# dlilien/ImpDAR

Measured on NVIDIA B200. Metric: migrated samples/s, higher is better.
Workload: dtype f32

## Files before the change

### impdar_b200/csrc/kirchhoff_tile.cuh

```cuda
#pragma once

namespace impdar {

#ifndef KT_CFG_NW
#define KT_CFG_NW 28
#endif
#ifndef KT_CFG_NP
#define KT_CFG_NP 4
#endif
#ifndef KT_CFG_RW
#define KT_CFG_RW 1
#endif
#ifndef KT_CFG_TR
#define KT_CFG_TR 8
#endif
#ifndef KT_CFG_W
#define KT_CFG_W 16
#endif
#ifndef KT_CFG_NST
#define KT_CFG_NST 4
#endif
constexpr int KT_NW = KT_CFG_NW;
constexpr int KT_NP = KT_CFG_NP;
constexpr int KT_RW = KT_CFG_RW;
constexpr int KT_Q = KT_NW * KT_RW;
constexpr int KT_TR = KT_CFG_TR;
constexpr int KT_X = 32 * KT_TR;
constexpr int KT_W = KT_CFG_W;
constexpr int KT_NST = KT_CFG_NST;
#ifndef KT_CFG_FLUSH
#define KT_CFG_FLUSH 4
#endif
constexpr int KT_FLUSH = KT_CFG_FLUSH;
constexpr int KT_SPAN = 120;
constexpr int KT_SEGW = KT_X + KT_SPAN + 8;
constexpr int KT_STAGE_FLOATS = KT_W * 2 * KT_SEGW;
constexpr int KT_RING = 33;
constexpr size_t KT_SMEM = (size_t)KT_NST * KT_STAGE_FLOATS * sizeof(float) +
                           (size_t)KT_NW * KT_RW * KT_RING * sizeof(int4) + 2 * KT_NST * sizeof(unsigned long long) + 16;
constexpr int KT_THREADS = (KT_NW + KT_NP) * 32;
constexpr int KT_RPP = (KT_W + KT_NP - 1) / KT_NP;
static_assert(KT_RPP <= 32 && KT_NW + KT_NP <= 32, "tile kernel configuration");

struct KirchTileParams {
    const int2 *seg;
    const int *nstage;
    int *sched_flags;
    int t_base;
};

struct KtPlace {
    long long gl, gr;
    unsigned nl, nr;
    int dl, dr;
    int ol, orr;
};
__device__ __forceinline__ KtPlace kt_place(const KirchTabParams &p, int x0, int k, int slot, int j, int2 e) {
    const int span = e.y - e.x;
    const long long rowoff = (long long)k * p.Tp + p.Apad + x0;
    const long long il = rowoff - e.y, ir = rowoff + e.x;
    const int shl = (int)(il & 3), shr = (int)(ir & 3);
    KtPlace r;
    r.gl = il - shl;
    r.gr = ir - shr;
    r.nl = (unsigned)((shl + KT_X + span + 3) & ~3);
    r.nr = (unsigned)((shr + KT_X + span + 3) & ~3);
    r.dl = slot * KT_STAGE_FLOATS + j * 2 * KT_SEGW;
    r.dr = r.dl + KT_SEGW;
    r.ol = r.dl + shl + e.y;
    r.orr = r.dr + shr - e.x;
    return r;
}

__device__ __forceinline__ unsigned kt_smem_u32(const void *p) { return (unsigned)__cvta_generic_to_shared(p); }
__device__ __forceinline__ void kt_mbar_init(unsigned long long *bar, int count) {
    asm volatile("mbarrier.init.shared::cta.b64 [%0], %1;" ::"r"(kt_smem_u32(bar)), "r"(count) : "memory");
}
__device__ __forceinline__ void kt_mbar_arrive(unsigned long long *bar) {
    asm volatile("mbarrier.arrive.shared::cta.b64 _, [%0];" ::"r"(kt_smem_u32(bar)) : "memory");
}
__device__ __forceinline__ void kt_mbar_arrive_tx(unsigned long long *bar, unsigned bytes) {
    asm volatile("mbarrier.arrive.expect_tx.shared::cta.b64 _, [%0], %1;" ::"r"(kt_smem_u32(bar)), "r"(bytes) : "memory");
}
#ifndef KT_CFG_SLEEP
#define KT_CFG_SLEEP 0
#endif
__device__ __forceinline__ bool kt_mbar_try(unsigned long long *bar, unsigned parity) {
    unsigned ok;
    asm volatile(
        "{\n"
        ".reg .pred p;\n"
        "mbarrier.try_wait.parity.shared::cta.b64 p, [%1], %2;\n"
        "selp.u32 %0, 1, 0, p;\n"
        "}\n"
        : "=r"(ok)
        : "r"(kt_smem_u32(bar)), "r"(parity)
        : "memory");
    return ok != 0;
}
__device__ __forceinline__ void kt_mbar_wait(unsigned long long *bar, unsigned parity) {
    while (!kt_mbar_try(bar, parity)) {
        if (KT_CFG_SLEEP) __nanosleep(KT_CFG_SLEEP);
    }
}
__device__ __forceinline__ void kt_bulk_load(void *smem_dst, const void *gsrc, unsigned bytes, unsigned long long *bar) {
    asm volatile("cp.async.bulk.shared::cluster.global.mbarrier::complete_tx::bytes [%0], [%1], %2, [%3];" ::"r"(
                     kt_smem_u32(smem_dst)),
                 "l"(gsrc), "r"(bytes), "r"(kt_smem_u32(bar))
                 : "memory");
}

__global__ void __launch_bounds__(256) kirch_tile_sched_kernel(const int2 *__restrict__ tab, const int *__restrict__ nm,
                                                               int S, int A1, int s_begin, int s_end, int2 *__restrict__ seg,
                                                               int *__restrict__ nstage, int *__restrict__ sched_flags) {
    __shared__ int s_kmax, s_wide;
    const int b = blockIdx.x;
    const int t0 = s_begin + b * KT_Q, t1 = min(t0 + KT_Q, s_end);
    int2 *__restrict__ sb = seg + (size_t)b * S;
    if (threadIdx.x == 0) { s_kmax = -1; s_wide = 0; }
    for (int k = t0 + threadIdx.x; k < S; k += blockDim.x) sb[k] = make_int2(0x7fffffff, -1);
    __syncthreads();
    int kmax = -1;
    for (int ti = t0; ti < t1; ++ti) {
        const int n = nm[ti];
        const int2 *__restrict__ row = tab + (size_t)ti * A1;
        for (int m = threadIdx.x; m < n; m += blockDim.x) {
            const int k = row[m].x;
            if (k >= 0) {
                atomicMin(&sb[k].x, m);
                atomicMax(&sb[k].y, m);
                kmax = max(kmax, k);
            }
        }
    }
    if (kmax >= 0) atomicMax(&s_kmax, kmax);
    __syncthreads();
    int wide = 0;
    for (int k = t0 + threadIdx.x; k < S; k += blockDim.x) {
        const int2 e = sb[k];
        if (e.y >= e.x && e.y - e.x > KT_SPAN) wide = 1;
    }
    if (wide) atomicOr(&s_wide, 1);
    __syncthreads();
    if (threadIdx.x == 0) {
        const int kbase = (t0 / KT_W) * KT_W;
        nstage[b] = s_kmax < 0 ? 0 : (s_kmax - kbase) / KT_W + 1;
        if (s_wide) atomicOr(sched_flags, 1);
    }
}

__global__ void __launch_bounds__(256) kirch_table_count_kernel(const int2 *__restrict__ tab, const int *__restrict__ nm,
                                                                int A1, int T, int x_begin, int x_end, int s_begin,
                                                                unsigned long long *__restrict__ stats) {
    const int ti = s_begin + blockIdx.x;
    const int n = nm[ti];
    const int2 *__restrict__ row = tab + (size_t)ti * A1;
    unsigned long long c = 0;
    for (int m = threadIdx.x; m < n; m += blockDim.x) {
        if (row[m].x < 0) continue;
        c += (unsigned long long)max(0, x_end - max(x_begin, m));
        if (m) c += (unsigned long long)max(0, min(x_end, T - m) - x_begin);
    }
#pragma unroll
    for (int o = 16; o > 0; o >>= 1) c += __shfl_xor_sync(0xffffffffu, c, o);
    if ((threadIdx.x & 31) == 0 && c) atomicAdd(&stats[0], c);
}

__global__ void __launch_bounds__(KT_THREADS, 1) kirch_tile_kernel(const __grid_constant__ KirchTabParams p,
                                                                   const __grid_constant__ KirchTileParams q) {
    extern __shared__ __align__(128) unsigned char kt_smem_raw[];
    if (q.sched_flags[0] != 0) return;
    const int b = blockIdx.x;
    const int t0 = q.t_base + b * KT_Q;
    const int r_lo = max(t0, p.flags[0]);
    if (min(t0 + KT_Q, p.s_end) <= r_lo) return;
    float *buf = reinterpret_cast<float *>(kt_smem_raw);
    int4 *rings = reinterpret_cast<int4 *>(buf + (size_t)KT_NST * KT_STAGE_FLOATS);
    unsigned long long *full = reinterpret_cast<unsigned long long *>(rings + KT_NW * KT_RW * KT_RING);
    unsigned long long *empty = full + KT_NST;

    const int x0 = p.x_begin + blockIdx.y * KT_X;
    const int nst = q.nstage[b];
    const int kbase = (t0 / KT_W) * KT_W;
    const int warp = threadIdx.x >> 5, lane = threadIdx.x & 31;
    const int2 *__restrict__ sb = q.seg + (size_t)b * p.S;

    if (threadIdx.x == 0) {
        for (int i = 0; i < KT_NST; ++i) {
            kt_mbar_init(&full[i], KT_NP);
            kt_mbar_init(&empty[i], KT_NW);
        }
        asm volatile("fence.mbarrier_init.release.cluster;" ::: "memory");
    }
    __syncthreads();

    if (warp >= KT_NW) {
        const int pw = warp - KT_NW;
        for (int s = 0; s < nst; ++s) {
            const int slot = s % KT_NST;
            if (s >= KT_NST) kt_mbar_wait(&empty[slot], (unsigned)((s / KT_NST - 1) & 1));
            unsigned bytes = 0, nl = 0, nr = 0;
            const float *gl = nullptr, *gr = nullptr;
            float *dl = nullptr, *dr = nullptr;
            const int j = pw * KT_RPP + lane;
            if (lane < KT_RPP && j < KT_W) {
                const int k = kbase + s * KT_W + j;
                int2 e = make_int2(1, 0);
                if (k >= t0 && k < p.S) e = sb[k];
                if (e.y >= e.x) {
                    const KtPlace pl = kt_place(p, x0, k, slot, j, e);
                    nl = pl.nl;
                    nr = pl.nr;
                    gl = p.gP + pl.gl;
                    gr = p.gP + pl.gr;
                    dl = buf + pl.dl;
                    dr = buf + pl.dr;
                    bytes = (nl + nr) * 4u;
                }
            }
            const unsigned total = __reduce_add_sync(0xffffffffu, bytes);
            __syncwarp();
            if (lane == 0) kt_mbar_arrive_tx(&full[slot], total);
            __syncwarp();
            if (bytes) {
                kt_bulk_load(dl, gl, nl * 4u, &full[slot]);
                kt_bulk_load(dr, gr, nr * 4u, &full[slot]);
            }
        }
        return;
    }

    float2 acc[KT_RW][KT_TR / 2], tot[KT_RW][KT_TR / 2];
    int mnext[KT_RW], mend[KT_RW];
    int pos[KT_RW], cnt[KT_RW];
    int csk[KT_RW];
    bool live[KT_RW];
    const int2 *trow[KT_RW];
    int2 pre[KT_RW];
    int4 *ring[KT_RW];
    int4 cur[KT_RW];
    const int2 none = make_int2(-1, 0);
    auto decode = [&](int w) {
        const int m = mnext[w] + lane;
        const int2 e = pre[w];
        pre[w] = m + 32 < mend[w] ? __ldg(trow[w] + m + 32) : none;
        const unsigned v = __ballot_sync(0xffffffffu, e.x >= 0);
        __syncwarp();
        csk[w] = 0x7fffffff;
        if (e.x >= 0) {
            const unsigned rel = (unsigned)(e.x - kbase), sk = rel / KT_W;
            const KtPlace pl = kt_place(p, x0, e.x, (int)(sk % KT_NST), (int)(rel % KT_W), __ldg(sb + e.x));
            const float wgt = __int_as_float(e.y) * (m == 0 ? 0.5f : 1.0f);
            ring[w][__popc(v & ((1u << lane) - 1u))] =
                make_int4((pl.ol - m) * 4, (pl.orr + m) * 4, __float_as_int(wgt), 0);
            csk[w] = (int)sk;
        }
        __syncwarp();
        mnext[w] += 32;
        pos[w] = 0;
        cnt[w] = __popc(v);
        cur[w] = ring[w][0];
    };
#pragma unroll
    for (int w = 0; w < KT_RW; ++w) {
        const int ti = t0 + warp + w * KT_NW;
        live[w] = ti >= max(p.s_begin, r_lo) && ti < p.s_end && (x0 < p.x_end);
        mnext[w] = 0;
        mend[w] = live[w] ? p.nm[ti] : 0;
        trow[w] = p.tab + (size_t)(live[w] ? ti : t0) * p.A1;
        ring[w] = rings + (size_t)(warp * KT_RW + w) * KT_RING;
        pre[w] = lane < mend[w] ? __ldg(trow[w] + lane) : none;
        decode(w);
#pragma unroll
        for (int r = 0; r < KT_TR / 2; ++r) acc[w][r] = tot[w][r] = make_float2(0.f, 0.f);
    }
    const char *__restrict__ lbuf = reinterpret_cast<const char *>(buf + lane);
    const int sabs0 = kbase / KT_W;
    for (int s = 0; s < nst; ++s) {
        const int slot = s % KT_NST;
        kt_mbar_wait(&full[slot], (unsigned)((s / KT_NST) & 1));
#pragma unroll
        for (int w = 0; w < KT_RW; ++w) {
            while (true) {
                const int end = __popc(__ballot_sync(0xffffffffu, csk[w] <= s));
                int4 d = cur[w];
#pragma unroll 1
                for (int i = pos[w]; i < end; ++i) {
                    const int4 nx = ring[w][i + 1];
                    const float *__restrict__ pl = reinterpret_cast<const float *>(lbuf + d.x);
                    const float *__restrict__ pr = reinterpret_cast<const float *>(lbuf + d.y);
                    const float wgt = __int_as_float(d.z);
                    const float2 w2 = make_float2(wgt, wgt);
#pragma unroll
                    for (int r = 0; r < KT_TR / 2; ++r) {
                        const float2 l = make_float2(pl[64 * r], pl[64 * r + 32]);
                        const float2 g = make_float2(pr[64 * r], pr[64 * r + 32]);
                        acc[w][r] = __ffma2_rn(w2, __fadd2_rn(l, g), acc[w][r]);
                    }
                    d = nx;
                }
                cur[w] = d;
                pos[w] = end;
                if (end < cnt[w] || mnext[w] >= mend[w]) break;
                decode(w);
            }
        }
        if (((sabs0 + s) & (KT_FLUSH - 1)) == KT_FLUSH - 1) {
#pragma unroll
            for (int w = 0; w < KT_RW; ++w)
#pragma unroll
                for (int r = 0; r < KT_TR / 2; ++r) {
                    tot[w][r] = __fadd2_rn(tot[w][r], acc[w][r]);
                    acc[w][r] = make_float2(0.f, 0.f);
                }
        }
        __syncwarp();
        if (lane == 0) kt_mbar_arrive(&empty[slot]);
    }
#pragma unroll
    for (int w = 0; w < KT_RW; ++w) {
        const int ti = t0 + warp + w * KT_NW;
        if (!live[w]) continue;
#pragma unroll
        for (int r = 0; r < KT_TR / 2; ++r) {
            const float2 v = __fadd2_rn(tot[w][r], acc[w][r]);
            const int x = x0 + lane + 64 * r;
            if (x < p.x_end) p.out[(size_t)ti * p.ldo + (x - p.x_begin)] = v.x;
            if (x + 32 < p.x_end) p.out[(size_t)ti * p.ldo + (x + 32 - p.x_begin)] = v.y;
        }
    }
}

}
```

Measured before the change: 3.523 billion.

## Pair adjacent output rows per warp to share identical shared-memory tap reads

Each consumer warp now handles two adjacent output traces (14 warps × 2 rows instead of 28 × 1). While decoding, it marks each tap entry whose trace index matches the neighbouring row's entry at the same offset. Matching taps are then processed together, with one shared-memory load feeding two FMAs, and non-matching runs are unrolled by two. This is meant to cut shared-memory bandwidth and instruction count per accumulation, at the cost of fewer warps for latency hiding, more register pressure and more complex control flow.

```diff
diff --git a/impdar_b200/csrc/kirchhoff_tile.cuh b/impdar_b200/csrc/kirchhoff_tile.cuh
--- a/impdar_b200/csrc/kirchhoff_tile.cuh
+++ b/impdar_b200/csrc/kirchhoff_tile.cuh
@@ -2,15 +2,9 @@
 
 namespace impdar {
 
-#ifndef KT_CFG_NW
-#define KT_CFG_NW 28
-#endif
 #ifndef KT_CFG_NP
 #define KT_CFG_NP 4
 #endif
-#ifndef KT_CFG_RW
-#define KT_CFG_RW 1
-#endif
 #ifndef KT_CFG_TR
 #define KT_CFG_TR 8
 #endif
@@ -20,10 +14,9 @@
 #ifndef KT_CFG_NST
 #define KT_CFG_NST 4
 #endif
-constexpr int KT_NW = KT_CFG_NW;
+constexpr int KT_NW = 14;
 constexpr int KT_NP = KT_CFG_NP;
-constexpr int KT_RW = KT_CFG_RW;
-constexpr int KT_Q = KT_NW * KT_RW;
+constexpr int KT_Q = 2 * KT_NW;
 constexpr int KT_TR = KT_CFG_TR;
 constexpr int KT_X = 32 * KT_TR;
 constexpr int KT_W = KT_CFG_W;
@@ -35,9 +28,9 @@
 constexpr int KT_SPAN = 120;
 constexpr int KT_SEGW = KT_X + KT_SPAN + 8;
 constexpr int KT_STAGE_FLOATS = KT_W * 2 * KT_SEGW;
-constexpr int KT_RING = 33;
+constexpr int KT_RING = 34;
 constexpr size_t KT_SMEM = (size_t)KT_NST * KT_STAGE_FLOATS * sizeof(float) +
-                           (size_t)KT_NW * KT_RW * KT_RING * sizeof(int4) + 2 * KT_NST * sizeof(unsigned long long) + 16;
+                           (size_t)KT_NW * 2 * KT_RING * sizeof(int4) + 2 * KT_NST * sizeof(unsigned long long) + 16;
 constexpr int KT_THREADS = (KT_NW + KT_NP) * 32;
 constexpr int KT_RPP = (KT_W + KT_NP - 1) / KT_NP;
 static_assert(KT_RPP <= 32 && KT_NW + KT_NP <= 32, "tile kernel configuration");
@@ -176,7 +169,7 @@
     if (min(t0 + KT_Q, p.s_end) <= r_lo) return;
     float *buf = reinterpret_cast<float *>(kt_smem_raw);
     int4 *rings = reinterpret_cast<int4 *>(buf + (size_t)KT_NST * KT_STAGE_FLOATS);
-    unsigned long long *full = reinterpret_cast<unsigned long long *>(rings + KT_NW * KT_RW * KT_RING);
+    unsigned long long *full = reinterpret_cast<unsigned long long *>(rings + KT_NW * 2 * KT_RING);
     unsigned long long *empty = full + KT_NST;
 
     const int x0 = p.x_begin + blockIdx.y * KT_X;
@@ -230,20 +223,23 @@
         return;
     }
 
-    float2 acc[KT_RW][KT_TR / 2], tot[KT_RW][KT_TR / 2];
-    int mnext[KT_RW], mend[KT_RW];
-    int pos[KT_RW], cnt[KT_RW];
-    int csk[KT_RW];
-    bool live[KT_RW];
-    const int2 *trow[KT_RW];
-    int2 pre[KT_RW];
-    int4 *ring[KT_RW];
-    int4 cur[KT_RW];
+    float2 acc[2][KT_TR / 2], tot[2][KT_TR / 2];
+    int mnext[2], mend[2];
+    int pos[2], cnt[2];
+    int csk[2];
+    const int2 *trow[2];
+    int2 pre[2];
+    int prek[2];
+    int4 *ring[2];
+    int4 cur[2];
+    bool live[2];
     const int2 none = make_int2(-1, 0);
     auto decode = [&](int w) {
         const int m = mnext[w] + lane;
         const int2 e = pre[w];
+        const int ko = prek[w];
         pre[w] = m + 32 < mend[w] ? __ldg(trow[w] + m + 32) : none;
+        prek[w] = m + 32 < mend[1 - w] ? __ldg(&trow[1 - w][m + 32].x) : -1;
         const unsigned v = __ballot_sync(0xffffffffu, e.x >= 0);
         __syncwarp();
         csk[w] = 0x7fffffff;
@@ -252,7 +248,7 @@
             const KtPlace pl = kt_place(p, x0, e.x, (int)(sk % KT_NST), (int)(rel % KT_W), __ldg(sb + e.x));
             const float wgt = __int_as_float(e.y) * (m == 0 ? 0.5f : 1.0f);
             ring[w][__popc(v & ((1u << lane) - 1u))] =
-                make_int4((pl.ol - m) * 4, (pl.orr + m) * 4, __float_as_int(wgt), 0);
+                make_int4((pl.ol - m) * 4, (pl.orr + m) * 4, __float_as_int(wgt), e.x == ko);
             csk[w] = (int)sk;
         }
         __syncwarp();
@@ -262,52 +258,99 @@
         cur[w] = ring[w][0];
     };
 #pragma unroll
-    for (int w = 0; w < KT_RW; ++w) {
-        const int ti = t0 + warp + w * KT_NW;
+    for (int w = 0; w < 2; ++w) {
+        const int ti = t0 + 2 * warp + w;
         live[w] = ti >= max(p.s_begin, r_lo) && ti < p.s_end && (x0 < p.x_end);
         mnext[w] = 0;
         mend[w] = live[w] ? p.nm[ti] : 0;
         trow[w] = p.tab + (size_t)(live[w] ? ti : t0) * p.A1;
-        ring[w] = rings + (size_t)(warp * KT_RW + w) * KT_RING;
+        ring[w] = rings + (size_t)(warp * 2 + w) * KT_RING;
+#pragma unroll
+        for (int r = 0; r < KT_TR / 2; ++r) acc[w][r] = tot[w][r] = make_float2(0.f, 0.f);
+    }
+#pragma unroll
+    for (int w = 0; w < 2; ++w) {
         pre[w] = lane < mend[w] ? __ldg(trow[w] + lane) : none;
+        prek[w] = lane < mend[1 - w] ? __ldg(&trow[1 - w][lane].x) : -1;
         decode(w);
-#pragma unroll
-        for (int r = 0; r < KT_TR / 2; ++r) acc[w][r] = tot[w][r] = make_float2(0.f, 0.f);
     }
     const char *__restrict__ lbuf = reinterpret_cast<const char *>(buf + lane);
     const int sabs0 = kbase / KT_W;
     for (int s = 0; s < nst; ++s) {
         const int slot = s % KT_NST;
         kt_mbar_wait(&full[slot], (unsigned)((s / KT_NST) & 1));
-#pragma unroll
-        for (int w = 0; w < KT_RW; ++w) {
-            while (true) {
-                const int end = __popc(__ballot_sync(0xffffffffu, csk[w] <= s));
-                int4 d = cur[w];
+        while (true) {
+            const int end0 = __popc(__ballot_sync(0xffffffffu, csk[0] <= s));
+            const int end1 = __popc(__ballot_sync(0xffffffffu, csk[1] <= s));
+            auto run = [&](int w, int end) {
+                int4 d = cur[w], nx = ring[w][pos[w] + 1];
+                int i = pos[w];
 #pragma unroll 1
-                for (int i = pos[w]; i < end; ++i) {
-                    const int4 nx = ring[w][i + 1];
+                while (i < end && !d.w) {
                     const float *__restrict__ pl = reinterpret_cast<const float *>(lbuf + d.x);
                     const float *__restrict__ pr = reinterpret_cast<const float *>(lbuf + d.y);
-                    const float wgt = __int_as_float(d.z);
-                    const float2 w2 = make_float2(wgt, wgt);
-#pragma unroll
-                    for (int r = 0; r < KT_TR / 2; ++r) {
-                        const float2 l = make_float2(pl[64 * r], pl[64 * r + 32]);
-                        const float2 g = make_float2(pr[64 * r], pr[64 * r + 32]);
-                        acc[w][r] = __ffma2_rn(w2, __fadd2_rn(l, g), acc[w][r]);
+                    const float2 w2 = make_float2(__int_as_float(d.z), __int_as_float(d.z));
+                    float2 lg[KT_TR / 2];
+#pragma unroll
+                    for (int r = 0; r < KT_TR / 2; ++r)
+                        lg[r] = __fadd2_rn(make_float2(pl[64 * r], pl[64 * r + 32]), make_float2(pr[64 * r], pr[64 * r + 32]));
+                    if (i + 1 < end && !nx.w) {
+                        const int4 n2 = ring[w][i + 2], n3 = ring[w][i + 3];
+                        const float *__restrict__ ql = reinterpret_cast<const float *>(lbuf + nx.x);
+                        const float *__restrict__ qr = reinterpret_cast<const float *>(lbuf + nx.y);
+                        const float2 v2 = make_float2(__int_as_float(nx.z), __int_as_float(nx.z));
+                        float2 lh[KT_TR / 2];
+#pragma unroll
+                        for (int r = 0; r < KT_TR / 2; ++r)
+                            lh[r] = __fadd2_rn(make_float2(ql[64 * r], ql[64 * r + 32]), make_float2(qr[64 * r], qr[64 * r + 32]));
+#pragma unroll
+                        for (int r = 0; r < KT_TR / 2; ++r) acc[w][r] = __ffma2_rn(w2, lg[r], acc[w][r]);
+#pragma unroll
+                        for (int r = 0; r < KT_TR / 2; ++r) acc[w][r] = __ffma2_rn(v2, lh[r], acc[w][r]);
+                        d = n2;
+                        nx = n3;
+                        i += 2;
+                    } else {
+                        const int4 n2 = ring[w][i + 2];
+#pragma unroll
+                        for (int r = 0; r < KT_TR / 2; ++r) acc[w][r] = __ffma2_rn(w2, lg[r], acc[w][r]);
+                        d = nx;
+                        nx = n2;
+                        i += 1;
                     }
-                    d = nx;
                 }
                 cur[w] = d;
-                pos[w] = end;
-                if (end < cnt[w] || mnext[w] >= mend[w]) break;
-                decode(w);
+                pos[w] = i;
+            };
+#pragma unroll 1
+            while (true) {
+                run(0, end0);
+                run(1, end1);
+                if (pos[0] >= end0 || pos[1] >= end1) break;
+                const int4 d = cur[0];
+                const float2 a2 = make_float2(__int_as_float(d.z), __int_as_float(d.z));
+                const float2 b2 = make_float2(__int_as_float(cur[1].z), __int_as_float(cur[1].z));
+                const float *__restrict__ pl = reinterpret_cast<const float *>(lbuf + d.x);
+                const float *__restrict__ pr = reinterpret_cast<const float *>(lbuf + d.y);
+                cur[0] = ring[0][++pos[0]];
+                cur[1] = ring[1][++pos[1]];
+#pragma unroll
+                for (int r = 0; r < KT_TR / 2; ++r) {
+                    const float2 lg = __fadd2_rn(make_float2(pl[64 * r], pl[64 * r + 32]),
+                                                 make_float2(pr[64 * r], pr[64 * r + 32]));
+                    acc[0][r] = __ffma2_rn(a2, lg, acc[0][r]);
+                    acc[1][r] = __ffma2_rn(b2, lg, acc[1][r]);
+                }
             }
+            const bool r0 = pos[0] == cnt[0] && mnext[0] < mend[0];
+            const bool r1 = pos[1] == cnt[1] && mnext[1] < mend[1];
+            if (!r0 && !r1) break;
+            if (r0) decode(0);
+            if (r1) decode(1);
         }
         if (((sabs0 + s) & (KT_FLUSH - 1)) == KT_FLUSH - 1) {
 #pragma unroll
-            for (int w = 0; w < KT_RW; ++w)
+            for (int w = 0; w < 2; ++w)
 #pragma unroll
                 for (int r = 0; r < KT_TR / 2; ++r) {
                     tot[w][r] = __fadd2_rn(tot[w][r], acc[w][r]);
@@ -318,8 +361,8 @@
         if (lane == 0) kt_mbar_arrive(&empty[slot]);
     }
 #pragma unroll
-    for (int w = 0; w < KT_RW; ++w) {
-        const int ti = t0 + warp + w * KT_NW;
+    for (int w = 0; w < 2; ++w) {
+        const int ti = t0 + 2 * warp + w;
         if (!live[w]) continue;
 #pragma unroll
         for (int r = 0; r < KT_TR / 2; ++r) {
```

Result: slower. 3.050 billion (median of 6 runs) (-13.4%).
